# nurturenature/jepsen-tigerbeetle

Measured on AMD Instinct MI355X. Metric: histories/sec, 10k-op/64-proc cas-register histories (time-to-verdict ms in extra), higher is better.
Workload: dtype u64

## Files before the change

### jepsen-tigerbeetle_amd/csrc/open_walk_impl.h

```cpp
#pragma once
#include "wave_env.h"
#include "tbc_internal.h"

namespace tbc {
namespace walk {

constexpr uint32_t kCandCap = 136;
constexpr uint32_t kCandWords = 8;
constexpr uint32_t kAuxWords = 80;
constexpr uint32_t kKeyWords = 32, kKeyBits = 32 * kKeyWords;
static_assert(2 * kKeyWords <= kAuxWords && kKeyWords == 32, "the map and its prefix fit the scratch; two rows of 16 lanes scan it");
WV_HD constexpr uint32_t walk_lds_words() { return kCandCap * kCandWords + kAuxWords; }

constexpr uint32_t kCList = 1u;
constexpr uint32_t kCTwin = 2u;
constexpr uint32_t kCRow = 4u;
constexpr uint32_t kCLook = 8u;

WV_DEV void or_slot(uint32_t& lo, uint32_t& hi, bool cond, uint32_t slot) {
  if (slot < 32u) lo = wv::opaque(lo | (cond ? (1u << slot) : 0u));
  else hi = wv::opaque(hi | (cond ? (1u << (slot - 32u)) : 0u));
}
WV_DEV uint32_t effect_key(uint32_t f, int32_t a, int32_t b) {
  return (f & 3u) | (((uint32_t)a & 0x7FFFu) << 2) | ((f == TBC_F_CAS ? ((uint32_t)b & 0x7FFFu) : 0u) << 17);
}
static_assert(kMaxRuleValue < 0x7FFF && TBC_F_READ < 3 && TBC_F_WRITE < 3 && TBC_F_CAS < 3, "effect_key packs f and two rule values into a word, and no key has all bits set");
static_assert(kLookNone <= 0xFFu, "the produced value shares a word with the flags");

WV_DEV uint32_t rank_code(uint32_t slot, uint32_t f, int32_t a, uint32_t vpad) {
  const uint32_t k8 = f == TBC_F_READ ? (rdm_index(a, vpad) & 0xFFu) : 0xFFu;
  return (slot & 63u) | ((k8 == 0xFFu ? 7u : (k8 & 7u)) << 6);
}

template <int Q>
WV_DEV void store_entries(const wv::u32x16& r, uint64_t* row, uint32_t n) {
  WV_UNROLL
  for (int v = 0; v < 8; v++) if ((uint32_t)(8 * Q + v) < n) row[8 * Q + v] = (uint64_t)r[2 * v] | ((uint64_t)r[2 * v + 1] << 32);
}

template <int VCAP>
WV_DEV void walk_wave(const PackOpenArgs& A, uint32_t wid, uint32_t* lds, uint32_t lane) {
  const uint32_t cph = A.chunks_per_hist;
  const uint32_t hr = wid / cph, c = wid - hr * cph, h = A.h0 + hr;
  if (h >= A.n_hist) return;
  const Hist* H = &A.hist[h];
  const BeamHist* B = &A.bh[h];
  const uint32_t R = H->n_ret;
  const uint32_t F_lo = c * 64u;
  if (H->status != 0 || B->status != 0 || F_lo >= R) return;
  const uint32_t F_hi = F_lo + 64u < R ? F_lo + 64u : R;
  const uint32_t W = H->n_slots;
  const Rec* rec = A.rec + H->rec_off;
  const uint32_t* seg = A.seg + H->seg_off;
  const uint32_t* off = A.off + B->off_off;
  OpRec* lst = A.lst + B->lst_off;
  uint64_t* twn = A.twn ? A.twn + B->lst_off : nullptr;
  const uint32_t V = A.vpad;
  const uint32_t FW = A.front_words ? A.front_words : V;
  const bool compact = A.front_compact != 0u;
  uint64_t* rdm = (A.rdm && (V || compact)) ? A.rdm + H->op_off * FW : nullptr;
  const bool want_tw = twn != nullptr;
  uint64_t* look = A.look ? A.look + look_off(H->op_off, h, 1u) : nullptr;
  uint32_t* cand = lds;
  uint32_t* aux = lds + kCandCap * kCandWords;

  const uint32_t ret_from = look ? (F_lo >= kLookahead - 1u ? F_lo - (kLookahead - 1u) : 0u) : F_lo;
  uint32_t lo = 0, k = 0;
  if (lane < W) {
    uint32_t l = seg[lane] + 1u, hi = seg[lane + 1] - 1u;
    const uint32_t tail = hi;
    while (l < hi) {
      const uint32_t mid = (l + hi) >> 1;
      if (rec[mid].ret_rank >= ret_from) hi = mid; else l = mid + 1u;
    }
    lo = l;
    uint32_t i = lo;
    for (;;) {
      const uint32_t i1 = i + 1u < tail ? i + 1u : tail, i2 = i + 2u < tail ? i + 2u : tail, i3 = i + 3u < tail ? i + 3u : tail;
      const uint32_t v0 = rec[i < tail ? i : tail].inv_rank, v1 = rec[i1].inv_rank, v2 = rec[i2].inv_rank, v3 = rec[i3].inv_rank;
      if (v0 >= F_hi) break;
      i++;
      if (v1 >= F_hi) break;
      i++;
      if (v2 >= F_hi) break;
      i++;
      if (v3 >= F_hi) break;
      i++;
    }
    k = i - lo;
  }
  uint32_t incl = k;
  for (uint32_t d = 1; d < 64u; d <<= 1) {
    aux[lane] = incl;
    wv::barrier();
    const uint32_t add = lane >= d ? aux[lane - d] : 0u;
    wv::barrier();
    incl += add;
  }
  const uint32_t base = incl - k;
  const uint32_t NC_all = wv::readlane(incl, 63u);
  const uint32_t NC = NC_all < kCandCap ? NC_all : kCandCap;
  for (uint32_t j = 0; j < k; j++) {
    const Rec r = rec[lo + j];
    if (base + j < kCandCap) {
      const bool live = (r.cls & 2u) != 0u, isread = (r.cls & 16u) != 0u, wc = (r.cls & 8u) != 0u;
      const bool in_chunk = r.ret_rank >= F_lo;
      const bool listed = live && in_chunk && !(A.branch_lists && isread);
      const uint32_t vi = rdm_index(r.a, V);
      uint32_t fl = (lane << 12) | (r.prod << 24);
      if (listed) fl |= kCList;
      if (listed && wc && want_tw) fl |= kCTwin;
      if (live && in_chunk && isread && rdm && V && (vi != 0u || r.a == TBC_NIL)) fl |= kCRow | (vi << 4);
      if (look && (r.cls & 6u) && r.prod != kLookNone) fl |= kCLook;
      uint32_t* e = cand + (base + j) * kCandWords;
      e[0] = r.inv_rank; e[1] = r.ret_rank; e[2] = r.opidx; e[3] = r.f | (lane << 8);
      e[4] = (uint32_t)r.a; e[5] = (uint32_t)r.b; e[6] = fl;
      e[7] = (live && wc && in_chunk) ? effect_key(r.f, r.a, r.b) : 0xFFFFFFFFu;
    }
  }
  wv::barrier();

  const uint32_t list_order = A.order_of ? A.order_of[h] : A.list_order;
  const bool by_ret = list_order != 0u;
  const uint32_t wr_last = list_order == 2u ? 0x40000000u : list_order >= 16u ? 2u * (list_order - 16u) + 1u : 0u;
  const uint32_t rk_mul = list_order >= 16u ? 2u : 1u;
  uint16_t* const perm = reinterpret_cast<uint16_t*>(aux);
  if (by_ret) {
    uint32_t my[3], place[3] = {0u, 0u, 0u};
    uint32_t d[3];
    const uint32_t wr_ofs = list_order == 2u ? kKeyBits / 2u : wr_last, lim_other = list_order == 2u ? kKeyBits / 2u : kKeyBits;
    bool outside = false;
    WV_UNROLL
    for (int s = 0; s < 3; s++) {
      const uint32_t idx = lane + 64u * (uint32_t)s;
      const uint32_t* e = cand + (idx < NC ? idx : 0u) * kCandWords;
      const uint32_t rt = e[1];
      const bool wr = (e[3] & 0xFFu) == TBC_F_WRITE;
      my[s] = idx >= NC ? 0xFFFFFFFFu : rt == kInf ? (0xFFFFFF00u | idx) : rt * rk_mul + (wr ? wr_last : 0u);
      const bool live = idx < NC && rt != kInf;
      const uint32_t x = rt - ret_from;
      const bool inside = x < kKeyBits && x * rk_mul + (wr ? wr_ofs : 0u) < (wr ? kKeyBits : lim_other);
      d[s] = (live && inside) ? x * rk_mul + (wr ? wr_ofs : 0u) : kInf;
      outside = outside || (live && !inside);
    }
    const uint32_t n0 = NC < 64u ? NC : 64u, n1 = NC <= 64u ? 0u : (NC < 128u ? NC - 64u : 64u), n2 = NC <= 128u ? 0u : NC - 128u;
    if (wr_ofs < kKeyBits && wv::ballot(outside) == 0ull) {
      if (lane < kKeyWords) aux[lane] = 0u;
      wv::barrier();
      WV_UNROLL
      for (int s = 0; s < 3; s++) if (d[s] != kInf) wv::lds_add32(&aux[d[s] >> 5], 1u << (d[s] & 31u));
      wv::barrier();
      const uint32_t wc = lane < kKeyWords ? (uint32_t)__builtin_popcount(aux[lane]) : 0u;
      uint32_t y = wc;
      y += wv::row_shr0<1>(y); y += wv::row_shr0<2>(y); y += wv::row_shr0<4>(y); y += wv::row_shr0<8>(y);
      const uint32_t row0 = wv::readlane(y, 15u);
      y += lane >= 16u ? row0 : 0u;
      const uint32_t n_live = wv::readlane(y, kKeyWords - 1u);
      if (lane < kKeyWords) aux[kKeyWords + lane] = y - wc;
      const uint64_t below = (1ull << lane) - 1ull;
      uint32_t cr_before = n_live;
      WV_UNROLL
      for (int s = 0; s < 3; s++) {
        const uint32_t idx = lane + 64u * (uint32_t)s;
        const uint64_t cr = wv::ballot(idx < NC && d[s] == kInf);
        if (d[s] == kInf) place[s] = cr_before + (uint32_t)__builtin_popcountll(cr & below);
        cr_before += (uint32_t)__builtin_popcountll(cr);
      }
      wv::barrier();
      WV_UNROLL
      for (int s = 0; s < 3; s++)
        if (d[s] != kInf) place[s] = aux[kKeyWords + (d[s] >> 5)] + (uint32_t)__builtin_popcount(aux[d[s] >> 5] & ((1u << (d[s] & 31u)) - 1u));
      wv::barrier();
    } else if (NC <= 64u) {
      for (uint32_t j = 0; j < n0; j++) place[0] += wv::readlane(my[0], j) < my[0] ? 1u : 0u;
    } else if (NC <= 128u) {
      for (uint32_t j = 0; j < n0; j++) { const uint32_t kj = wv::readlane(my[0], j); place[0] += kj < my[0] ? 1u : 0u; place[1] += kj < my[1] ? 1u : 0u; }
      for (uint32_t j = 0; j < n1; j++) { const uint32_t kj = wv::readlane(my[1], j); place[0] += kj < my[0] ? 1u : 0u; place[1] += kj < my[1] ? 1u : 0u; }
    } else {
      WV_UNROLL
      for (int s2 = 0; s2 < 3; s2++) {
        const uint32_t cnt = s2 == 0 ? n0 : s2 == 1 ? n1 : n2;
        for (uint32_t j = 0; j < cnt; j++) {
          const uint32_t kj = wv::readlane(my[s2], j);
          place[0] += kj < my[0] ? 1u : 0u; place[1] += kj < my[1] ? 1u : 0u; place[2] += kj < my[2] ? 1u : 0u;
        }
      }
    }
    WV_UNROLL
    for (int s = 0; s < 3; s++) {
      const uint32_t idx = lane + 64u * (uint32_t)s;
      if (idx < NC) perm[place[s]] = (uint16_t)idx;
    }
    wv::barrier();
  }

  uint32_t c_key[3] = {0xFFFFFFFFu, 0xFFFFFFFFu, 0xFFFFFFFFu}, c_ret[3] = {0u, 0u, 0u};
  if (want_tw) {
    WV_UNROLL
    for (int s = 0; s < 3; s++) {
      const uint32_t idx = lane + 64u * (uint32_t)s;
      const uint32_t* e = cand + (idx < NC ? idx : 0u) * kCandWords;
      c_key[s] = idx < NC ? e[7] : 0xFFFFFFFFu;
      c_ret[s] = e[1];
    }
  }

  const uint32_t F = F_lo + lane;
  const bool active = F < F_hi;
  const uint32_t Fc = active ? F : F_hi - 1u;
  const uint32_t pos0 = off[Fc];
  uint32_t pos = pos0;
  const uint32_t px = A.ret_slot[H->ret_off + Fc];
  uint32_t need = kLookNone, xprod = kLookNone, di = 0, x = 0, xf = kFNone;
  int32_t xa = 0;
  if (look || compact) {
    x = A.ret_op[H->ret_off + Fc];
    xf = A.f[H->op_off + x];
    xa = A.a[H->op_off + x];
  }
  if (look) {
    const int32_t xb = A.b[H->op_off + x];
    const uint32_t xinv = A.scratch[H->frame_off + x];
    need = look_need(xf, xa); xprod = look_prod(xf, xa, xb);
    di = F - xinv < 255u ? F - xinv : 255u;
  }
  wv::u32x16 r0, r1, r2, r3;
  WV_UNROLL
  for (int i = 0; i < 16; i++) { r0[i] = 0u; r1[i] = 0u; r2[i] = 0u; r3[i] = 0u; }
  uint32_t pm_lo = 0u, pm_hi = 0u, dmin = 255u;

  WV_NOUNROLL
  for (uint32_t t = 0; t < NC; t++) {
    const uint32_t* e = cand + (by_ret ? (uint32_t)perm[t] : t) * kCandWords;
    const uint32_t inv = e[0], ret = e[1];
    const uint32_t fl = wv::readfirstlane(e[6]);
    const uint32_t slot = (fl >> 12) & 63u;
    const bool member = active && inv <= F && F <= ret;
    if (fl & kCList) {
      uint32_t tw_lo = 0u, tw_hi = 0u;
      if (fl & kCTwin) {
        const uint32_t key_t = e[7];
        uint64_t s0 = wv::ballot(c_key[0] == key_t && c_ret[0] < ret && c_ret[0] >= inv);
        uint64_t s1 = 0ull, s2 = 0ull;
        if (NC > 64u) s1 = wv::ballot(c_key[1] == key_t && c_ret[1] < ret && c_ret[1] >= inv);
        if (NC > 128u) s2 = wv::ballot(c_key[2] == key_t && c_ret[2] < ret && c_ret[2] >= inv);
        while (s0 | s1 | s2) {
          uint32_t u;
          if (s0) { u = (uint32_t)__builtin_ctzll(s0); s0 &= s0 - 1ull; }
          else if (s1) { u = 64u + (uint32_t)__builtin_ctzll(s1); s1 &= s1 - 1ull; }
          else { u = 128u + (uint32_t)__builtin_ctzll(s2); s2 &= s2 - 1ull; }
          const uint32_t* eu = cand + u * kCandWords;
          const bool mu = eu[0] <= F && F <= eu[1];
          or_slot(tw_lo, tw_hi, mu, (wv::readfirstlane(eu[6]) >> 12) & 63u);
        }
      }
      if (member) {
        OpRec o; o.op = e[2]; o.f_slot = e[3] | (ret == F ? kAtFront : 0u); o.a = (int32_t)e[4]; o.b = (int32_t)e[5];
        lst[pos] = o;
        if (twn) twn[pos] = (uint64_t)tw_lo | ((uint64_t)tw_hi << 32);
        pos++;
      }
    }
    if (fl & kCRow)
    {
      const uint32_t w = ((fl >> 4) & 31u) * 2u + (slot >> 5), bit = member ? (1u << (slot & 31u)) : 0u;
      if constexpr (VCAP <= 8) r0[w & 15u] |= bit;
      else {
        const uint32_t q = w >> 4;
        if (q == 0u) r0[w & 15u] |= bit; else if (q == 1u) r1[w & 15u] |= bit; else if (q == 2u) r2[w & 15u] |= bit; else r3[w & 15u] |= bit;
      }
    }
    if (fl & kCLook) {
      const bool hit = (fl >> 24) == need;
      or_slot(pm_lo, pm_hi, member && hit, slot);
      const uint32_t dist = F - inv;
      if (hit && dist < kLookahead && e[2] != x) dmin = dist < dmin ? dist : dmin;
    }
  }

  uint64_t w6 = 0ull, w7 = 0ull;
  if (compact) {
    if (by_ret) wv::barrier();
    aux[lane] = active ? rank_code(px, xf, xa, V) : (7u << 6);
    if (lane < kFrontCompactRanks - 1u) {
      const uint32_t G = F_lo + 64u + lane;
      uint32_t code = 7u << 6;
      if (G < R) {
        const uint32_t gx = A.ret_op[H->ret_off + G];
        code = rank_code(A.ret_slot[H->ret_off + G], A.f[H->op_off + gx], A.a[H->op_off + gx], V);
      }
      aux[64u + lane] = code;
    }
    wv::barrier();
    WV_UNROLL
    for (uint32_t l = 0; l < kFrontCompactRanks; l++) w7 |= (uint64_t)aux[lane + l] << (9u * l);
    const uint32_t nl = pos - pos0, nc = A.ncr[B->off_off + Fc];
    w6 = (uint64_t)pos0 | ((uint64_t)(nl & 0xFFu) << 32) | ((uint64_t)((nl + nc) & 0xFFFFFFu) << 40);
  }
  if (!active) return;
  if (rdm) {
    uint64_t* row = rdm + (uint64_t)F * FW;
    const uint32_t n_row = compact ? 6u : V;
    store_entries<0>(r0, row, n_row);
    if constexpr (VCAP > 8) { store_entries<1>(r1, row, n_row); store_entries<2>(r2, row, n_row); store_entries<3>(r3, row, n_row); }
    if (compact) { row[6] = w6; row[7] = w7; }
  }
  if (look) {
    uint64_t pm = (uint64_t)pm_lo | ((uint64_t)pm_hi << 32);
    pm &= ~(1ull << (px & 63u));
    const uint64_t w0 = (uint64_t)(px & 0xFFFFu) | (uint64_t)need << 16 | (uint64_t)xprod << 24 | (uint64_t)di << 32 | ((uint64_t)dmin << 40);
    look[(uint64_t)F * 2u] = w0;
    look[(uint64_t)F * 2u + 1u] = pm;
  }
}

}
}
```

### jepsen-tigerbeetle_amd/csrc/pack_open.hip

```cpp
#include <hip/hip_runtime.h>
#include <cstdlib>
#include <cstring>
#include "tbc_internal.h"
#include "open_walk_impl.h"

namespace tbc {

namespace {

__device__ __forceinline__ uint32_t ld_agent(const uint32_t* p) {
  return __hip_atomic_load(p, __ATOMIC_RELAXED, __HIP_MEMORY_SCOPE_AGENT);
}
__device__ __forceinline__ uint64_t ld_agent64(const uint64_t* p) {
  return __hip_atomic_load(p, __ATOMIC_RELAXED, __HIP_MEMORY_SCOPE_AGENT);
}

__device__ __forceinline__ void scan_parts(uint32_t* part, uint32_t NT, uint32_t* total_slot) {
  if (threadIdx.x < 64) {
    const uint32_t lane = threadIdx.x, per = NT / 64, lo = lane * per;
    uint32_t sum = 0;
    for (uint32_t i = 0; i < per; i++) sum += part[lo + i];
    uint32_t x = sum;
    for (uint32_t d = 1; d < 64; d <<= 1) { const uint32_t y = __shfl_up(x, d); if (lane >= d) x += y; }
    uint32_t run = x - sum;
    for (uint32_t i = 0; i < per; i++) { const uint32_t v = part[lo + i]; part[lo + i] = run; run += v; }
    if (lane == 63 && total_slot) *total_slot = x;
  }
}

constexpr uint32_t kBatch = 8;
template <class F>
__device__ __forceinline__ void chunk_loads(const uint32_t* p, uint32_t lo, uint32_t hi, F&& each) {
  for (uint32_t i = lo; i < hi; i += kBatch) {
    uint32_t v[kBatch];
#pragma unroll
    for (uint32_t k = 0; k < kBatch; k++) v[k] = i + k < hi ? ld_agent(&p[i + k]) : 0u;
#pragma unroll
    for (uint32_t k = 0; k < kBatch; k++) if (i + k < hi) each(i + k, v[k]);
  }
}

}

__global__ __launch_bounds__(1024) void open_counts_kernel(PackOpenArgs A) {
  __shared__ uint32_t s_part[1024];
  const uint32_t NT = blockDim.x;
  __shared__ uint32_t s_total;
  const uint32_t tid = threadIdx.x;
  const uint32_t MW = A.mask_words;

  for (uint32_t h = A.h0 + blockIdx.x; h < A.n_hist; h += gridDim.x) {
    const Hist* H = &A.hist[h];
    BeamHist* B = &A.bh[h];
    const uint32_t n = H->n_ops, R = H->n_ret;
    if (H->status != 0 || R == 0) {
      if (tid == 0) { B->status = 0; B->n_crashed = 0; B->lst_need = 0; }
      continue;
    }
    const bool cf = (H->flags & kHistCount) != 0u;
    const uint8_t* f = A.f + H->op_off;
    const int32_t* a = A.a + H->op_off;
    const int32_t* b = A.b + H->op_off;
    const int32_t* proc = A.process + H->op_off;
    const uint32_t* sc_inv = A.scratch + H->frame_off;
    const uint32_t* sc_ret = sc_inv + n;
    uint32_t* off = A.off + B->off_off;
    uint32_t* ncr = A.ncr + B->off_off;
    OpRec* crashed = A.crashed + H->op_off;
    const uint32_t* ret_slot = A.ret_slot + H->ret_off;
    uint8_t* slot8 = A.slot8 + slot8_off(H->op_off, h);

    for (uint32_t r = tid; r < R + 16u; r += NT) slot8[r] = r < R ? (uint8_t)ret_slot[r] : (uint8_t)0;
    if (A.rk8) {
      uint8_t* rk8 = A.rk8 + slot8_off(H->op_off, h);
      const uint32_t* ret_op = A.ret_op + H->ret_off;
      for (uint32_t r = tid; r < R + 16u; r += NT) {
        uint8_t k = 0xFF;
        if (r < R) { const uint32_t x = ret_op[r]; if (f[x] == TBC_F_READ) k = (uint8_t)rdm_index(a[x], A.vpad); }
        rk8[r] = k;
      }
    }
    for (uint32_t i0 = tid; i0 < n; i0 += 4u * NT) {
      uint32_t ir[4], rr[4]; bool nilread[4], isread[4];
#pragma unroll
      for (uint32_t k = 0; k < 4; k++) {
        const uint32_t i = i0 + k * NT;
        const bool in = i < n;
        ir[k] = in ? sc_inv[i] : 0u; rr[k] = in ? sc_ret[i] : 0u;
        isread[k] = in && f[i] == TBC_F_READ;
        nilread[k] = isread[k] && a[i] == TBC_NIL;
      }
#pragma unroll
      for (uint32_t k = 0; k < 4; k++) {
        if (i0 + k * NT >= n) continue;
        if (rr[k] == kInf) {
          if (!cf && ir[k] < R && !nilread[k]) atomicAdd(&ncr[ir[k]], 1u);
        } else if (!(A.branch_lists && isread[k])) {
          atomicAdd(&off[ir[k]], 1u);
        }
      }
    }
    __syncthreads();
    uint32_t total;
    {
      const uint32_t chunk = (R + NT - 1) / NT;
      const uint32_t lo = min(tid * chunk, R), hi = min(lo + chunk, R);
      uint64_t rdbits = 0;
      uint32_t base_rd = 0;
      if (A.branch_lists) {
        const uint8_t* rk8 = A.rk8 + slot8_off(H->op_off, h);
        uint32_t nrd = 0;
        if (hi - lo <= 64u) { for (uint32_t i = lo; i < hi; i++) if (rk8[i] != 0xFFu) rdbits |= 1ull << (i - lo); nrd = (uint32_t)__popcll(rdbits); }
        else for (uint32_t i = lo; i < hi; i++) nrd += rk8[i] != 0xFFu;
        s_part[tid] = nrd;
        __syncthreads();
        scan_parts(s_part, NT, nullptr);
        __syncthreads();
        base_rd = s_part[tid];
        __syncthreads();
      }
      const bool wide_chunk = hi - lo > 64u;
      const uint8_t* rk8w = A.rk8 ? A.rk8 + slot8_off(H->op_off, h) : nullptr;
      const auto rd_at = [&](uint32_t i) -> uint32_t {
        if (!A.branch_lists) return 0u;
        return wide_chunk ? (uint32_t)(rk8w[i] != 0xFFu) : (uint32_t)((rdbits >> (i - lo)) & 1ull);
      };
      uint32_t sum = 0;
      chunk_loads(off, lo, hi, [&](uint32_t, uint32_t v) { sum += v; });
      s_part[tid] = sum;
      __syncthreads();
      scan_parts(s_part, NT, nullptr);
      __syncthreads();
      const uint32_t base_inv = s_part[tid];
      __syncthreads();
      uint32_t run = base_inv, open_sum = 0, rd = base_rd;
      chunk_loads(off, lo, hi, [&](uint32_t i, uint32_t v) { run += v; open_sum += run - (i - rd); rd += rd_at(i); });
      s_part[tid] = open_sum;
      __syncthreads();
      scan_parts(s_part, NT, &s_total);
      __syncthreads();
      uint32_t pos = s_part[tid];
      run = base_inv; rd = base_rd;
      chunk_loads(off, lo, hi, [&](uint32_t i, uint32_t v) { run += v; off[i] = pos; pos += run - (i - rd); rd += rd_at(i); });
      total = s_total;
      if (tid == 0) off[R] = total;
      __syncthreads();
    }
    {
      const uint32_t chunk = (R + NT - 1) / NT;
      const uint32_t lo = min(tid * chunk, R), hi = min(lo + chunk, R);
      uint32_t sum = 0;
      chunk_loads(ncr, lo, hi, [&](uint32_t, uint32_t v) { sum += v; });
      s_part[tid] = sum;
      __syncthreads();
      scan_parts(s_part, NT, nullptr);
      __syncthreads();
      uint32_t run = s_part[tid];
      chunk_loads(ncr, lo, hi, [&](uint32_t i, uint32_t v) { run += v; ncr[i] = run; });
      __syncthreads();
    }
    if (tid == 0) B->lst_need = total;
    if (total > B->lst_cap) {
      if (tid == 0) { B->status = 1; B->n_crashed = 0; }
      __syncthreads();
      continue;
    }
    if (cf) {
      if (tid == 0) { B->n_crashed = 0; B->status = 0; }
      __syncthreads();
    } else {
      const uint32_t chunk = (n + NT - 1) / NT;
      const uint32_t lo = min(tid * chunk, n), hi = min(lo + chunk, n);
      const bool small = hi - lo <= 64u;
      uint64_t mine = 0;
      uint32_t cnt = 0;
      if (small) {
        for (uint32_t i = lo; i < hi; i += kBatch) {
          uint32_t rr[kBatch]; uint8_t ff[kBatch]; int32_t aa[kBatch];
#pragma unroll
          for (uint32_t k = 0; k < kBatch; k++) { const bool in = i + k < hi; rr[k] = in ? sc_ret[i + k] : 0u; ff[k] = in ? f[i + k] : (uint8_t)0; aa[k] = in ? a[i + k] : 0; }
#pragma unroll
          for (uint32_t k = 0; k < kBatch; k++)
            if (i + k < hi && rr[k] == kInf && !(ff[k] == TBC_F_READ && aa[k] == TBC_NIL)) mine |= 1ull << (i + k - lo);
        }
        cnt = (uint32_t)__popcll(mine);
      } else {
        for (uint32_t i = lo; i < hi; i++) cnt += sc_ret[i] == kInf && !(f[i] == TBC_F_READ && a[i] == TBC_NIL);
      }
      s_part[tid] = cnt;
      __syncthreads();
      scan_parts(s_part, NT, &s_total);
      __syncthreads();
      if (tid == 0) { B->n_crashed = s_total; B->status = 0; }
      uint32_t run = s_part[tid];
      if (small) {
        while (mine) {
          const uint32_t i = lo + (uint32_t)__builtin_ctzll(mine);
          mine &= mine - 1ull;
          OpRec o; o.op = i; o.f_slot = (uint32_t)f[i] | ((uint32_t)proc[i] << 8); o.a = a[i]; o.b = b[i];
          crashed[run++] = o;
        }
      } else {
        for (uint32_t i = lo; i < hi; i++) if (sc_ret[i] == kInf && !(f[i] == TBC_F_READ && a[i] == TBC_NIL)) {
          OpRec o; o.op = i; o.f_slot = (uint32_t)f[i] | ((uint32_t)proc[i] << 8); o.a = a[i]; o.b = b[i];
          crashed[run++] = o;
        }
      }
      __syncthreads();
    }
    if (A.look) {
      const uint32_t LW = 1 + MW;
      uint64_t* look = A.look + look_off(H->op_off, h, MW);
      for (uint32_t t = R + tid; t < R + kLookPad; t += NT) {
        look[(uint64_t)t * LW] = (uint64_t)(kLookNone << 16 | kLookNone << 24) | (255ull << 32) | (255ull << 40);
        for (uint32_t w = 0; w < MW; w++) look[(uint64_t)t * LW + 1 + w] = 0ull;
      }
    }
  }
}

namespace {
struct Cur { uint32_t inv, ret, op, f; int32_t a, b; uint32_t cls, prod; };
__device__ __forceinline__ Cur load_cur(const Rec* r) {
  const Rec x = *r;
  return Cur{x.inv_rank, x.ret_rank, x.opidx, x.f, x.a, x.b, x.cls, x.prod};
}
}

template <int MW>
__global__ __launch_bounds__(256) void open_walk_kernel(PackOpenArgs A) {
  const uint32_t lane = threadIdx.x & 63u;
  const uint32_t wid = blockIdx.x * 4u + (threadIdx.x >> 6);
  const uint32_t cph = A.chunks_per_hist;
  const uint32_t hr = wid / cph, c = wid - hr * cph, h = A.h0 + hr;
  if (h >= A.n_hist) return;
  const Hist* H = &A.hist[h];
  const BeamHist* B = &A.bh[h];
  const uint32_t R = H->n_ret;
  const uint32_t F_lo = c * 64u;
  if (H->status != 0 || B->status != 0 || F_lo >= R) return;
  const uint32_t F_hi = min(F_lo + 64u, R);
  const uint32_t W = H->n_slots;
  const Rec* rec = A.rec + H->rec_off;
  const uint32_t* seg = A.seg + H->seg_off;
  const uint32_t* off = A.off + B->off_off;
  OpRec* lst = A.lst + B->lst_off;
  const uint32_t* ret_slot = A.ret_slot + H->ret_off;
  uint64_t* twn = A.twn ? A.twn + B->lst_off * MW : nullptr;
  const uint32_t V = A.vpad;
  const uint32_t FW = A.front_words ? A.front_words : V * MW;
  uint64_t* rdm = A.rdm ? A.rdm + H->op_off * FW : nullptr;
  uint64_t* look = A.look ? A.look + look_off(H->op_off, h, MW) : nullptr;
  uint32_t* tmp = A.tmp ? A.tmp + H->op_off : nullptr;

  Cur cur[MW], nxt[MW];
  uint32_t at[MW], tail[MW];
#pragma unroll
  for (int j = 0; j < MW; j++) {
    const uint32_t p = lane + 64u * (uint32_t)j;
    cur[j] = Cur{kInf, kInf, kInf, kFNone, 0, 0, 0u, kLookNone}; nxt[j] = cur[j]; at[j] = 0; tail[j] = 0;
    if (p < W) {
      uint32_t lo = seg[p] + 1u, hi = seg[p + 1] - 1u;
      tail[j] = hi;
      while (lo < hi) {
        const uint32_t mid = (lo + hi) >> 1;
        if (rec[mid].ret_rank >= F_lo) hi = mid; else lo = mid + 1u;
      }
      at[j] = lo;
      cur[j] = load_cur(rec + lo);
      nxt[j] = load_cur(rec + min(lo + 1u, tail[j]));
    }
  }
  const uint32_t w_off = off[min(F_lo + lane, R)];
  const uint32_t w_slot = ret_slot[min(F_lo + lane, R - 1u)];
  const uint64_t below = (1ull << lane) - 1ull;
  uint64_t tw[MW][MW];
  bool known[MW];
#pragma unroll
  for (int j = 0; j < MW; j++) {
    known[j] = false;
#pragma unroll
    for (int w = 0; w < MW; w++) tw[j][w] = 0ull;
  }

  for (uint32_t F = F_lo; F < F_hi; F++) {
    const uint32_t base = __builtin_amdgcn_readlane(w_off, F - F_lo);
    const uint32_t px = __builtin_amdgcn_readlane(w_slot, F - F_lo);
    bool live[MW], crashed_open[MW], inl[MW];
    uint64_t occ[MW];
#pragma unroll
    for (int j = 0; j < MW; j++) {
      const bool here = cur[j].inv <= F;
      live[j] = here && (cur[j].cls & 2u);
      crashed_open[j] = here && (cur[j].cls & 4u);
      inl[j] = live[j] && !(A.branch_lists && (cur[j].cls & 16u));
      occ[j] = __ballot(inl[j]);
    }
    uint32_t before = 0, mypos[MW];
#pragma unroll
    for (int j = 0; j < MW; j++) {
      mypos[j] = base + before + (uint32_t)__popcll(occ[j] & below);
      before += (uint32_t)__popcll(occ[j]);
      if (inl[j]) {
        OpRec o; o.op = cur[j].op; o.f_slot = cur[j].f | ((lane + 64u * (uint32_t)j) << 8) | (cur[j].ret == F ? kAtFront : 0u);
        o.a = cur[j].a; o.b = cur[j].b;
        lst[mypos[j]] = o;
      }
    }
    if (twn) {
#pragma unroll
      for (int jj = 0; jj < MW; jj++) {
        uint64_t m = __ballot(live[jj] && (cur[jj].cls & 8u) && !known[jj]);
        while (m) {
          const uint32_t l = (uint32_t)__builtin_ctzll(m);
          m &= m - 1ull;
          const uint32_t zf = __builtin_amdgcn_readlane(cur[jj].f, l), zr = __builtin_amdgcn_readlane(cur[jj].ret, l);
          const int32_t za = (int32_t)__builtin_amdgcn_readlane((uint32_t)cur[jj].a, l), zb = (int32_t)__builtin_amdgcn_readlane((uint32_t)cur[jj].b, l);
#pragma unroll
          for (int j = 0; j < MW; j++) {
            const bool same = live[j] && cur[j].f == zf && cur[j].a == za && (zf != TBC_F_CAS || cur[j].b == zb) && !(j == jj && lane == l);
            if (same && zr < cur[j].ret) tw[j][jj] |= 1ull << l;
            const uint64_t earlier = __ballot(same && cur[j].ret < zr);
            if (lane == l) tw[jj][j] = earlier;
          }
        }
      }
#pragma unroll
      for (int j = 0; j < MW; j++) {
        const bool wc = live[j] && (cur[j].cls & 8u);
        if (wc) known[j] = true;
        if (inl[j]) {
#pragma unroll
          for (int w = 0; w < MW; w++) twn[(uint64_t)mypos[j] * MW + w] = wc ? tw[j][w] : 0ull;
        }
      }
    }
    if (rdm) {
      uint64_t mine[MW];
#pragma unroll
      for (int j = 0; j < MW; j++) mine[j] = 0ull;
#pragma unroll
      for (int j = 0; j < MW; j++) {
        uint64_t rd = __ballot(live[j] && (cur[j].cls & 16u));
        while (rd) {
          const uint32_t l = (uint32_t)__builtin_ctzll(rd);
          rd &= rd - 1ull;
          const int32_t va = (int32_t)__builtin_amdgcn_readlane((uint32_t)cur[j].a, l);
          const uint32_t vi = rdm_index(va, V);
          if (lane == vi && (vi != 0u || va == TBC_NIL)) mine[j] |= 1ull << l;
        }
      }
      if (lane < V) {
#pragma unroll
        for (int j = 0; j < MW; j++) rdm[(uint64_t)F * FW + lane * MW + j] = mine[j];
      }
    }
    if (look) {
      const uint32_t jx = px >> 6, lx = px & 63u;
      uint32_t xf = kFNone, xinv = 0; int32_t xa = 0, xb = 0;
#pragma unroll
      for (int j = 0; j < MW; j++) if (jx == (uint32_t)j) {
        xf = __builtin_amdgcn_readlane(cur[j].f, lx); xinv = __builtin_amdgcn_readlane(cur[j].inv, lx);
        xa = (int32_t)__builtin_amdgcn_readlane((uint32_t)cur[j].a, lx); xb = (int32_t)__builtin_amdgcn_readlane((uint32_t)cur[j].b, lx);
      }
      const uint32_t need = look_need(xf, xa), prod = look_prod(xf, xa, xb), di = min(F - xinv, 255u);
      const uint64_t w0 = (uint64_t)(px & 0xFFFFu) | (uint64_t)need << 16 | (uint64_t)prod << 24 | (uint64_t)di << 32 | (255ull << 40);
      const uint32_t LW = 1 + MW;
#pragma unroll
      for (int j = 0; j < MW; j++) {
        const bool other = (live[j] || crashed_open[j]) && !(jx == (uint32_t)j && lane == lx);
        const uint64_t pm = need == kLookNone ? 0ull : __ballot(other && cur[j].prod == need);
        if (lane == 0) look[(uint64_t)F * LW + 1 + j] = pm;
      }
      if (lane == 0) { look[(uint64_t)F * LW] = w0; tmp[F] = 255u; }
    }
#pragma unroll
    for (int j = 0; j < MW; j++) {
      if (twn) {
#pragma unroll
        for (int w = 0; w < MW; w++) if ((px >> 6) == (uint32_t)w) tw[j][w] &= ~(1ull << (px & 63u));
      }
      if ((px >> 6) == (uint32_t)j && lane == (px & 63u)) {
        if (twn) {
#pragma unroll
          for (int w = 0; w < MW; w++) tw[j][w] = 0ull;
          known[j] = false;
        }
        cur[j] = nxt[j];
        at[j] = min(at[j] + 1u, tail[j]);
        nxt[j] = load_cur(rec + min(at[j] + 1u, tail[j]));
      }
    }
  }
}

template <int VCAP>
__global__ __launch_bounds__(256, 2) void open_walk_fronts_kernel(PackOpenArgs A) {
  extern __shared__ __attribute__((aligned(16))) uint32_t walk_lds[];
  const uint32_t lane = threadIdx.x & 63u;
  const uint32_t wv_ = (uint32_t)__builtin_amdgcn_readfirstlane((int)(threadIdx.x >> 6));
  walk::walk_wave<VCAP>(A, blockIdx.x * 4u + wv_, walk_lds + wv_ * walk::walk_lds_words(), lane);
}

__global__ __launch_bounds__(1024) void open_dprod_kernel(PackOpenArgs A) {
  const uint32_t NT = blockDim.x, tid = threadIdx.x, MW = A.mask_words;
  for (uint32_t h = A.h0 + blockIdx.x; h < A.n_hist; h += gridDim.x) {
    const Hist* H = &A.hist[h];
    const BeamHist* B = &A.bh[h];
    const uint32_t n = H->n_ops, R = H->n_ret;
    if (H->status != 0 || B->status != 0 || R == 0) continue;
    const uint8_t* f = A.f + H->op_off;
    const int32_t* a = A.a + H->op_off;
    const int32_t* b = A.b + H->op_off;
    const uint32_t* sc_inv = A.scratch + H->frame_off;
    const uint32_t* sc_ret = sc_inv + n;
    const uint32_t LW = 1 + MW;
    uint64_t* look = A.look + look_off(H->op_off, h, MW);
    const uint32_t* ret_op = A.ret_op + H->ret_off;
    uint32_t* tmp = A.tmp + H->op_off;
    for (uint32_t i = tid; i < n; i += NT) {
      const uint32_t pv = look_prod(f[i], a[i], b[i]);
      if (pv == kLookNone || (sc_ret[i] == kInf && f[i] == TBC_F_READ)) continue;
      const uint32_t ir = sc_inv[i];
      uint64_t w[kLookahead]; uint32_t ro[kLookahead];
#pragma unroll
      for (uint32_t k = 0; k < kLookahead; k++) {
        const uint32_t t = ir + k;
        const bool in = t < R;
        w[k] = in ? ld_agent64(&look[(uint64_t)t * LW]) : 0ull;
        ro[k] = in ? ret_op[t] : 0u;
      }
#pragma unroll
      for (uint32_t k = 0; k < kLookahead; k++) {
        const uint32_t t = ir + k;
        if (t < R && ((uint32_t)(w[k] >> 16) & 0xFFu) == pv && ro[k] != i) atomicMin(&tmp[t], k);
      }
    }
    __syncthreads();
    for (uint32_t t0 = tid; t0 < R; t0 += 4u * NT) {
      uint32_t d[4]; uint64_t w0[4];
#pragma unroll
      for (uint32_t k = 0; k < 4; k++) {
        const uint32_t t = t0 + k * NT;
        d[k] = t < R ? ld_agent(&tmp[t]) : 255u;
        w0[k] = t < R ? ld_agent64(&look[(uint64_t)t * LW]) : 0ull;
      }
#pragma unroll
      for (uint32_t k = 0; k < 4; k++) {
        const uint32_t t = t0 + k * NT;
        if (t < R && d[k] < 255u) look[(uint64_t)t * LW] = (w0[k] & ~(255ull << 40)) | ((uint64_t)d[k] << 40);
      }
    }
    __syncthreads();
  }
}

__global__ __launch_bounds__(256) void count_fronts_kernel(PackOpenArgs A, uint32_t phase) {
  const uint32_t NT = blockDim.x, tid = threadIdx.x, LW = 1u + A.mask_words;
  for (uint32_t h = A.h0 + blockIdx.x; h < A.n_hist; h += gridDim.x) {
    const Hist* H = &A.hist[h];
    const BeamHist* B = &A.bh[h];
    const uint32_t R = H->n_ret, nc = B->n_classes;
    if (!(H->flags & kHistCount) || H->status != 0 || B->status != 0 || R == 0 || nc == 0) continue;
    const uint64_t* cmem = A.cmem + B->cmem_off;
    const OpRec* cls = reinterpret_cast<const OpRec*>(cmem);
    uint32_t* ncr = A.ncr + B->off_off;
    uint64_t* look = (A.look && phase == 1u) ? A.look + look_off(H->op_off, h, A.mask_words) : nullptr;
    if (phase == 1u && !look) continue;
    for (uint32_t F = tid; F < R; F += NT) {
      const uint32_t need = look ? (uint32_t)(look[(uint64_t)F * LW] >> 16) & 0xFFu : kLookNone;
      uint32_t avail = 0; bool producer = false;
      for (uint32_t c = 0; c < nc; c++) {
        const OpRec o = cls[c];
        if ((uint32_t)cmem[o.op] > F) break;
        avail++;
        producer = producer || look_prod(o.f_slot & 0xFFu, o.a, o.b) == need;
      }
      if (phase == 0u) ncr[F] = avail;
      else if (producer && need != kLookNone) look[(uint64_t)F * LW] |= 1ull << 48;
    }
  }
}

__global__ __launch_bounds__(256) void front_meta_kernel(PackOpenArgs A) {
  const uint32_t cph = A.chunks_per_hist * 64u;
  const uint64_t gid = (uint64_t)blockIdx.x * 256u + threadIdx.x;
  const uint32_t hr = (uint32_t)(gid / cph), F = (uint32_t)(gid - (uint64_t)hr * cph), h = A.h0 + hr;
  if (h >= A.n_hist) return;
  const Hist* H = &A.hist[h];
  const BeamHist* B = &A.bh[h];
  if (H->status != 0 || B->status != 0 || F >= H->n_ret) return;
  const uint32_t* off = A.off + B->off_off;
  const uint32_t o0 = off[F], o1 = off[F + 1u], nc = A.ncr[B->off_off + F];
  const uint8_t* s8 = A.slot8 + slot8_off(H->op_off, h) + F;
  const uint8_t* k8 = A.rk8 + slot8_off(H->op_off, h) + F;
  uint64_t w[4] = {0, 0, 0, 0};
#pragma unroll
  for (uint32_t l = 0; l < 16; l++) {
    w[l >> 3] |= (uint64_t)s8[l] << (8u * (l & 7u));
    w[2 + (l >> 3)] |= (uint64_t)k8[l] << (8u * (l & 7u));
  }
  if (A.front_compact) {
    uint64_t* rec = A.rdm + (H->op_off + F) * kFrontCompactWords;
    uint64_t win = 0;
#pragma unroll
    for (uint32_t l = 0; l < kFrontCompactRanks; l++) {
      const uint32_t sl = (uint32_t)(w[0] >> (8u * l)) & 63u, k = (uint32_t)(w[2] >> (8u * l)) & 0xFFu;
      win |= (uint64_t)(sl | ((k == 0xFFu ? 7u : (k & 7u)) << 6)) << (9u * l);
    }
    rec[6] = (uint64_t)o0 | ((uint64_t)((o1 - o0) & 0xFFu) << 32) | ((uint64_t)(((o1 - o0) + nc) & 0xFFFFFFu) << 40);
    rec[7] = win;
    return;
  }
  uint64_t* rec = A.rdm + (H->op_off + F) * A.front_words + A.vpad * A.mask_words;
  rec[0] = (uint64_t)o0 | ((uint64_t)(o1 - o0) << 32);
  rec[1] = (uint64_t)((o1 - o0) + nc);
  rec[2] = w[0]; rec[3] = w[1]; rec[4] = w[2]; rec[5] = w[3];
}

void launch_open_counts(const PackOpenArgs& a, void* stream) {
  const uint32_t n_here = a.n_hist - a.h0;
  hipLaunchKernelGGL(open_counts_kernel, dim3(n_here < 4096 ? n_here : 4096), dim3(n_here <= 64 ? 1024 : 256), 0, (hipStream_t)stream, a);
}

void launch_pack_open(const PackOpenArgs& a, void* stream, bool skip_counts) {
  hipStream_t s = (hipStream_t)stream;
  const uint32_t n_here = a.n_hist - a.h0;
  const uint32_t grid = n_here < 4096 ? n_here : 4096;
  const uint32_t nt = n_here <= 64 ? 1024 : 256;
  if (!skip_counts) hipLaunchKernelGGL(open_counts_kernel, dim3(grid), dim3(nt), 0, s, a);
  if (a.cmem) hipLaunchKernelGGL(count_fronts_kernel, dim3(grid), dim3(256), 0, s, a, 0u);
  const uint64_t waves = (uint64_t)n_here * a.chunks_per_hist;
  const uint32_t wgrid = (uint32_t)((waves + 3) / 4);
  const bool by_front = a.mask_words == 1 && a.vpad <= 32;
  const size_t walk_lds_bytes = 4u * walk::walk_lds_words() * sizeof(uint32_t);
  if (by_front) {
    if (a.vpad <= 8) hipLaunchKernelGGL(open_walk_fronts_kernel<8>, dim3(wgrid), dim3(256), walk_lds_bytes, s, a);
    else hipLaunchKernelGGL(open_walk_fronts_kernel<32>, dim3(wgrid), dim3(256), walk_lds_bytes, s, a);
  } else switch (a.mask_words) {
    case 2: hipLaunchKernelGGL(open_walk_kernel<2>, dim3(wgrid), dim3(256), 0, s, a); break;
    default: hipLaunchKernelGGL(open_walk_kernel<4>, dim3(wgrid), dim3(256), 0, s, a); break;
  }
  if (a.look && !by_front) hipLaunchKernelGGL(open_dprod_kernel, dim3(grid), dim3(nt), 0, s, a);
  if (a.cmem) hipLaunchKernelGGL(count_fronts_kernel, dim3(grid), dim3(256), 0, s, a, 1u);
  if (a.front_words && !(by_front && a.front_compact)) {
    const uint64_t fronts = (uint64_t)n_here * a.chunks_per_hist * 64u;
    hipLaunchKernelGGL(front_meta_kernel, dim3((uint32_t)((fronts + 255) / 256)), dim3(256), 0, s, a);
  }
}

}
```

Measured before the change: 399,500.

## Walk runs of consecutive chunks per wavefront, carrying per-slot cursors in LDS

Each wavefront now processes a run of consecutive 64-return chunks of one history instead of a single chunk. The per-slot record cursor and the count of still-open records are kept in LDS, so later chunks skip the binary search for their first open record. The launch grid shrinks by the run length, and launch bounds rise to 8 blocks per CU for the small-VCAP variant, which forces register limits. In exchange the kernel loses parallelism for histories with few chunks, serializes chunks within a wave, and the scan bound is relaxed to the last record of the history.

After: 406,100 (median of 6 runs). +1.7%, better.

```diff
diff --git a/jepsen-tigerbeetle_amd/csrc/open_walk_impl.h b/jepsen-tigerbeetle_amd/csrc/open_walk_impl.h
--- a/jepsen-tigerbeetle_amd/csrc/open_walk_impl.h
+++ b/jepsen-tigerbeetle_amd/csrc/open_walk_impl.h
@@ -10,7 +10,9 @@
 constexpr uint32_t kAuxWords = 80;
 constexpr uint32_t kKeyWords = 32, kKeyBits = 32 * kKeyWords;
 static_assert(2 * kKeyWords <= kAuxWords && kKeyWords == 32, "the map and its prefix fit the scratch; two rows of 16 lanes scan it");
-WV_HD constexpr uint32_t walk_lds_words() { return kCandCap * kCandWords + kAuxWords; }
+constexpr uint32_t kCursorWords = 64 + 32;
+WV_HD constexpr uint32_t walk_lds_words() { return kCandCap * kCandWords + kAuxWords + kCursorWords; }
+static_assert(4u * walk_lds_words() * sizeof(uint32_t) <= 20u * 1024u, "eight blocks of four wavefronts a CU");
 
 constexpr uint32_t kCList = 1u;
 constexpr uint32_t kCTwin = 2u;
@@ -38,16 +40,43 @@
   for (int v = 0; v < 8; v++) if ((uint32_t)(8 * Q + v) < n) row[8 * Q + v] = (uint64_t)r[2 * v] | ((uint64_t)r[2 * v + 1] << 32);
 }
 
+#ifndef TBC_WALK_RUN
+#define TBC_WALK_RUN 8
+#endif
+constexpr uint32_t kWalkRun = TBC_WALK_RUN;
+static_assert(kWalkRun >= 1u, "a run has a chunk");
+constexpr uint32_t kStatWalkSearch = 40, kStatWalkCarried = 41, kStatWalkCursorMiss = 42;
+
+#if defined(TBC_EMU)
+WV_DEV uint32_t opaque_uniform(uint32_t v) { return v; }
+#else
+WV_DEV uint32_t opaque_uniform(uint32_t v) { asm volatile("" : "+s"(v)); return v; }
+#endif
+
+#if defined(TBC_EMU)
+template <class T>
+WV_DEV const T* read_only(const T* p) { return p; }
+#else
+template <class T>
+WV_DEV const __attribute__((address_space(4))) T* read_only(const T* p) { return (const __attribute__((address_space(4))) T*)(uintptr_t)p; }
+#endif
+
+WV_DEV uint32_t first_open(const Rec* rec, uint32_t l, uint32_t hi, uint32_t ret_from) {
+  while (l < hi) {
+    const uint32_t mid = (l + hi) >> 1;
+    if (rec[mid].ret_rank >= ret_from) hi = mid; else l = mid + 1u;
+  }
+  return l;
+}
+
 template <int VCAP>
-WV_DEV void walk_wave(const PackOpenArgs& A, uint32_t wid, uint32_t* lds, uint32_t lane) {
-  const uint32_t cph = A.chunks_per_hist;
-  const uint32_t hr = wid / cph, c = wid - hr * cph, h = A.h0 + hr;
-  if (h >= A.n_hist) return;
-  const Hist* H = &A.hist[h];
-  const BeamHist* B = &A.bh[h];
+WV_DEV bool walk_chunk(const PackOpenArgs& A_, uint32_t h, uint32_t c, uint32_t* lds, uint32_t lane, bool carried) {
+  const auto& A = *wv::cold(A_);
+  const auto* H = read_only(&A.hist[h]);
+  const auto* B = read_only(&A.bh[h]);
   const uint32_t R = H->n_ret;
   const uint32_t F_lo = c * 64u;
-  if (H->status != 0 || B->status != 0 || F_lo >= R) return;
+  if (H->status != 0 || B->status != 0 || F_lo >= R) return false;
   const uint32_t F_hi = F_lo + 64u < R ? F_lo + 64u : R;
   const uint32_t W = H->n_slots;
   const Rec* rec = A.rec + H->rec_off;
@@ -63,21 +92,28 @@
   uint64_t* look = A.look ? A.look + look_off(H->op_off, h, 1u) : nullptr;
   uint32_t* cand = lds;
   uint32_t* aux = lds + kCandCap * kCandWords;
+  uint32_t* const cur_end = aux + kAuxWords;
+  uint16_t* const cur_left = reinterpret_cast<uint16_t*>(cur_end + 64);
 
   const uint32_t ret_from = look ? (F_lo >= kLookahead - 1u ? F_lo - (kLookahead - 1u) : 0u) : F_lo;
+  const uint32_t ret_from_next = look ? F_lo + 64u - (kLookahead - 1u) : F_lo + 64u;
   uint32_t lo = 0, k = 0;
+  if (lane == 0u) wv::stat(carried ? kStatWalkCarried : kStatWalkSearch, 1);
   if (lane < W) {
-    uint32_t l = seg[lane] + 1u, hi = seg[lane + 1] - 1u;
-    const uint32_t tail = hi;
-    while (l < hi) {
-      const uint32_t mid = (l + hi) >> 1;
-      if (rec[mid].ret_rank >= ret_from) hi = mid; else l = mid + 1u;
-    }
-    lo = l;
-    uint32_t i = lo;
+    uint32_t i;
+    if (carried) { i = cur_end[lane]; lo = i - cur_left[lane]; }
+    else {
+      lo = first_open(rec, seg[lane] + 1u, seg[lane + 1] - 1u, ret_from);
+      i = lo;
+    }
+#if defined(TBC_EMU)
+    if (carried && lo != first_open(rec, seg[lane] + 1u, seg[lane + 1] - 1u, ret_from)) wv::stat(kStatWalkCursorMiss, 1);
+    if (i > seg[lane + 1] - 1u) wv::stat(kStatWalkCursorMiss, 1);
+#endif
+    const uint32_t last = read_only(seg)[W] - 1u;
     for (;;) {
-      const uint32_t i1 = i + 1u < tail ? i + 1u : tail, i2 = i + 2u < tail ? i + 2u : tail, i3 = i + 3u < tail ? i + 3u : tail;
-      const uint32_t v0 = rec[i < tail ? i : tail].inv_rank, v1 = rec[i1].inv_rank, v2 = rec[i2].inv_rank, v3 = rec[i3].inv_rank;
+      const uint32_t i1 = i + 1u < last ? i + 1u : last, i2 = i + 2u < last ? i + 2u : last, i3 = i + 3u < last ? i + 3u : last;
+      const uint32_t v0 = rec[i].inv_rank, v1 = rec[i1].inv_rank, v2 = rec[i2].inv_rank, v3 = rec[i3].inv_rank;
       if (v0 >= F_hi) break;
       i++;
       if (v1 >= F_hi) break;
@@ -100,8 +136,10 @@
   const uint32_t base = incl - k;
   const uint32_t NC_all = wv::readlane(incl, 63u);
   const uint32_t NC = NC_all < kCandCap ? NC_all : kCandCap;
+  uint32_t gone = 0;
   for (uint32_t j = 0; j < k; j++) {
     const Rec r = rec[lo + j];
+    gone += r.ret_rank < ret_from_next ? 1u : 0u;
     if (base + j < kCandCap) {
       const bool live = (r.cls & 2u) != 0u, isread = (r.cls & 16u) != 0u, wc = (r.cls & 8u) != 0u;
       const bool in_chunk = r.ret_rank >= F_lo;
@@ -118,6 +156,7 @@
       e[7] = (live && wc && in_chunk) ? effect_key(r.f, r.a, r.b) : 0xFFFFFFFFu;
     }
   }
+  cur_end[lane] = lo + k; cur_left[lane] = (uint16_t)(k - gone);
   wv::barrier();
 
   const uint32_t list_order = A.order_of ? A.order_of[h] : A.list_order;
@@ -297,22 +336,44 @@
     const uint32_t nl = pos - pos0, nc = A.ncr[B->off_off + Fc];
     w6 = (uint64_t)pos0 | ((uint64_t)(nl & 0xFFu) << 32) | ((uint64_t)((nl + nc) & 0xFFFFFFu) << 40);
   }
-  if (!active) return;
-  if (rdm) {
+  if (active && rdm) {
     uint64_t* row = rdm + (uint64_t)F * FW;
     const uint32_t n_row = compact ? 6u : V;
     store_entries<0>(r0, row, n_row);
     if constexpr (VCAP > 8) { store_entries<1>(r1, row, n_row); store_entries<2>(r2, row, n_row); store_entries<3>(r3, row, n_row); }
     if (compact) { row[6] = w6; row[7] = w7; }
   }
-  if (look) {
+  if (active && look) {
     uint64_t pm = (uint64_t)pm_lo | ((uint64_t)pm_hi << 32);
     pm &= ~(1ull << (px & 63u));
     const uint64_t w0 = (uint64_t)(px & 0xFFFFu) | (uint64_t)need << 16 | (uint64_t)xprod << 24 | (uint64_t)di << 32 | ((uint64_t)dmin << 40);
     look[(uint64_t)F * 2u] = w0;
     look[(uint64_t)F * 2u + 1u] = pm;
   }
-}
-
-}
-}
+  return F_lo + 64u < R;
+}
+
+template <int VCAP>
+WV_DEV void walk_wave(const PackOpenArgs& A, uint32_t wid, uint32_t* lds, uint32_t lane) {
+  const uint32_t cph = A.chunks_per_hist;
+  const uint32_t hr = wid / cph, c = wid - hr * cph, h = A.h0 + hr;
+  if (h >= A.n_hist) return;
+  (void)walk_chunk<VCAP>(A, h, c, lds, lane, false);
+}
+
+WV_HD constexpr uint32_t walk_runs_per_hist(uint32_t chunks_per_hist, uint32_t run = kWalkRun) { return (chunks_per_hist + run - 1u) / run; }
+
+template <int VCAP, uint32_t RUN = kWalkRun>
+WV_DEV void walk_run(const PackOpenArgs& A, uint32_t run_id, uint32_t* lds, uint32_t lane) {
+  const uint32_t rph = walk_runs_per_hist(A.chunks_per_hist, RUN);
+  const uint32_t hr = run_id / rph, c0 = (run_id - hr * rph) * RUN, h = A.h0 + hr;
+  if (h >= A.n_hist) return;
+  WV_NOUNROLL
+  for (uint32_t j = 0; j < RUN; j++) {
+    if (!walk_chunk<VCAP>(A, opaque_uniform(h), c0 + j, lds, wv::opaque(lane), j != 0u)) break;
+    wv::barrier();
+  }
+}
+
+}
+}
diff --git a/jepsen-tigerbeetle_amd/csrc/pack_open.hip b/jepsen-tigerbeetle_amd/csrc/pack_open.hip
--- a/jepsen-tigerbeetle_amd/csrc/pack_open.hip
+++ b/jepsen-tigerbeetle_amd/csrc/pack_open.hip
@@ -395,11 +395,11 @@
 }
 
 template <int VCAP>
-__global__ __launch_bounds__(256, 2) void open_walk_fronts_kernel(PackOpenArgs A) {
+__global__ __launch_bounds__(256, VCAP <= 8 ? 8 : 2) void open_walk_fronts_kernel(PackOpenArgs A) {
   extern __shared__ __attribute__((aligned(16))) uint32_t walk_lds[];
   const uint32_t lane = threadIdx.x & 63u;
   const uint32_t wv_ = (uint32_t)__builtin_amdgcn_readfirstlane((int)(threadIdx.x >> 6));
-  walk::walk_wave<VCAP>(A, blockIdx.x * 4u + wv_, walk_lds + wv_ * walk::walk_lds_words(), lane);
+  walk::walk_run<VCAP>(A, blockIdx.x * 4u + wv_, walk_lds + wv_ * walk::walk_lds_words(), lane);
 }
 
 __global__ __launch_bounds__(1024) void open_dprod_kernel(PackOpenArgs A) {
@@ -535,8 +535,10 @@
   const bool by_front = a.mask_words == 1 && a.vpad <= 32;
   const size_t walk_lds_bytes = 4u * walk::walk_lds_words() * sizeof(uint32_t);
   if (by_front) {
-    if (a.vpad <= 8) hipLaunchKernelGGL(open_walk_fronts_kernel<8>, dim3(wgrid), dim3(256), walk_lds_bytes, s, a);
-    else hipLaunchKernelGGL(open_walk_fronts_kernel<32>, dim3(wgrid), dim3(256), walk_lds_bytes, s, a);
+    const uint64_t runs = (uint64_t)n_here * walk::walk_runs_per_hist(a.chunks_per_hist);
+    const uint32_t rgrid = (uint32_t)((runs + 3) / 4);
+    if (a.vpad <= 8) hipLaunchKernelGGL(open_walk_fronts_kernel<8>, dim3(rgrid), dim3(256), walk_lds_bytes, s, a);
+    else hipLaunchKernelGGL(open_walk_fronts_kernel<32>, dim3(rgrid), dim3(256), walk_lds_bytes, s, a);
   } else switch (a.mask_words) {
     case 2: hipLaunchKernelGGL(open_walk_kernel<2>, dim3(wgrid), dim3(256), 0, s, a); break;
     default: hipLaunchKernelGGL(open_walk_kernel<4>, dim3(wgrid), dim3(256), 0, s, a); break;
```
